# TritonDataCenter/dragnet

Hardware: AMD Instinct MI355X
Metric: NDJSON records/sec (whole node), krill filter + 2-field breakdown (req.method,res.statusCode) (higher is better)
Workload: dtype uint8; 1 GPU; model=dn scan: filter eq(req.method,GET) + breakdown req.method,res.statusCode, global_batch=4743501, seq_len=226, parallelism=dp1

## Files before the change

### dragnet_amd/ops/hip/scan_record.h

```cpp
#pragma once
#include "scan_text.h"

namespace dn {

constexpr int BLOCK = 256;
constexpr int SIG_DEPTH = 6;


struct FV {
  uint8_t* type;
  uint32_t* soff;
  uint32_t* slen;
  int tid;
  DN_HD_INLINE void set(int f, uint8_t t, uint32_t off, uint32_t len,
                        double n) {
    type[f * BLOCK + tid] = t;
    if (t == T_NUM) {
      uint64_t b = (uint64_t)DN_DOUBLE_AS_LL(n);
      soff[f * BLOCK + tid] = (uint32_t)b;
      slen[f * BLOCK + tid] = (uint32_t)(b >> 32);
    } else {
      soff[f * BLOCK + tid] = off;
      slen[f * BLOCK + tid] = len;
    }
  }
  DN_HD_INLINE void set_len(int f, uint32_t len) {
    slen[f * BLOCK + tid] = len;
  }
  DN_HD_INLINE uint8_t get_type(int f) const { return type[f * BLOCK + tid]; }
  DN_HD_INLINE uint32_t get_soff(int f) const { return soff[f * BLOCK + tid]; }
  DN_HD_INLINE uint32_t get_slen(int f) const { return slen[f * BLOCK + tid]; }
  DN_HD_INLINE double get_num(int f) const {
    uint64_t b = (uint64_t)soff[f * BLOCK + tid]
               | ((uint64_t)slen[f * BLOCK + tid] << 32);
    return DN_LL_AS_DOUBLE((long long)b);
  }
};


template <class BS>
DN_HD_INLINE bool parse_record(BS BV, uint32_t start, uint32_t end,
                               const PlanView& P, FV& fv, uint8_t& top_type,
                               uint64_t* sig_lds, bool dot_splits) {
  CursorT<BS> c; c.init(BV, start, end);
  #define sig_stack_at(d) sig_lds[(d) * BLOCK + DN_TID()]

  uint64_t cont_slot = ~0ull;
  uint64_t is_arr_bits = 0;
  int depth = 0;
  int arr_depth = 0;
  uint64_t cur_sig = 0;
  bool cur_capture = false;
  int cur_slot = -1;

  c.skip_ws();
  if (c.eof()) return false;

  auto match_slot = [&](uint64_t sig) -> int {
    if (!((P.sig_bloom >> ((uint32_t)sig & 63u)) & 1ull)) return -1;
    for (int f = 0; f < P.nf; f++)
      if (P.field_sigs[f] == sig) return f;
    return -1;
  };

  auto parse_key = [&](uint64_t parent, bool root, uint64_t& sig_out) -> bool {
    if (c.eof() || c.next() != '"') return false;
    int r = scan_key_sig(c, root ? FNV_OFFSET : parent, sig_out,
                         dot_splits);
    if (r == 0) return false;
    if (r == 2 && !root && parent == P.fields_parent_sig)
      sig_out = sig_mix(sig_out ^ SIG_LIT_MARK);
    return true;
  };

  bool expect_value = true;
  top_type = T_MISSING;

  while (true) {
    if (expect_value) {
      c.skip_ws();
      if (c.eof()) return false;
      uint8_t b = c.peek();
      uint8_t vtype = T_MISSING;
      uint32_t voff = 0, vlen = 0;
      double vnum = 0.0;

      if (b == '{') {
        uint32_t vstart = c.pos;
        c.pos++;
        if (cur_capture && arr_depth == 0)
          fv.set(cur_slot, T_OBJ, vstart, 0, 0.0);
        if (depth == 0) top_type = T_OBJ;
        if (depth >= MAX_DEPTH) return false;
        c.skip_ws();
        if (!c.eof() && c.peek() == '}') {
          c.pos++;
          vtype = T_OBJ;
          voff = vstart; vlen = c.pos - vstart;
        } else {
          if (depth < SLOT_DEPTH) {
            uint64_t cs = (cur_capture && arr_depth == 0)
                              ? (uint64_t)cur_slot : 31ull;
            cont_slot = (cont_slot & ~(31ull << (5 * depth)))
                        | (cs << (5 * depth));
          }
          if (depth < SIG_DEPTH) sig_stack_at(depth) = cur_sig;
          is_arr_bits &= ~(1ull << depth);
          depth++;
          uint64_t ksig;
          if (!parse_key(cur_sig, depth == 1, ksig)) return false;
          c.skip_ws();
          if (c.eof() || c.next() != ':') return false;
          cur_sig = ksig;
          cur_slot = (arr_depth == 0) ? match_slot(ksig) : -1;
          cur_capture = cur_slot >= 0;
          continue;
        }
      } else if (b == '[') {
        uint32_t vstart = c.pos;
        c.pos++;
        if (cur_capture && arr_depth == 0)
          fv.set(cur_slot, T_ARR, vstart, 0, 0.0);
        if (depth == 0) top_type = T_ARR;
        if (depth >= MAX_DEPTH) return false;
        c.skip_ws();
        if (!c.eof() && c.peek() == ']') {
          c.pos++;
          vtype = T_ARR;
          voff = vstart; vlen = c.pos - vstart;
        } else {
          if (depth < SLOT_DEPTH) {
            uint64_t cs = (cur_capture && arr_depth == 0)
                              ? (uint64_t)cur_slot : 31ull;
            cont_slot = (cont_slot & ~(31ull << (5 * depth)))
                        | (cs << (5 * depth));
          }
          if (depth < SIG_DEPTH) sig_stack_at(depth) = cur_sig;
          is_arr_bits |= (1ull << depth);
          depth++;
          arr_depth++;
          cur_capture = false; cur_slot = -1;
          continue;
        }
      } else if (b == '"') {
        c.pos++;
        if (!scan_string_fast(c, voff, vlen)) return false;
        vtype = T_STR;
      } else if (b == 't') {
        if (c.end - c.pos < 4) return false;
        if (c.byte_at(c.pos+1)!='r'||c.byte_at(c.pos+2)!='u'||c.byte_at(c.pos+3)!='e') return false;
        c.pos += 4; vtype = T_TRUE;
      } else if (b == 'f') {
        if (c.end - c.pos < 5) return false;
        if (c.byte_at(c.pos+1)!='a'||c.byte_at(c.pos+2)!='l'||c.byte_at(c.pos+3)!='s'||c.byte_at(c.pos+4)!='e') return false;
        c.pos += 5; vtype = T_FALSE;
      } else if (b == 'n') {
        if (c.end - c.pos < 4) return false;
        if (c.byte_at(c.pos+1)!='u'||c.byte_at(c.pos+2)!='l'||c.byte_at(c.pos+3)!='l') return false;
        c.pos += 4; vtype = T_NULL;
      } else if (b == '-' || (b >= '0' && b <= '9')) {
        NumOut n = parse_json_number(c);
        if (!n.ok) return false;
        vtype = T_NUM; vnum = n.v;
      } else {
        return false;
      }

      if (vtype != T_MISSING) {
        if (cur_capture && arr_depth == 0)
          fv.set(cur_slot, vtype, voff, vlen, vnum);
        if (depth == 0) { top_type = (top_type == T_MISSING) ? vtype : top_type; }
      }
      expect_value = false;
      continue;
    }

    if (depth == 0) {
      c.skip_ws();
      return c.eof();
    }
    c.skip_ws();
    if (c.eof()) return false;
    uint8_t b = c.next();
    bool in_arr = (is_arr_bits >> (depth - 1)) & 1u;
    if (in_arr) {
      if (b == ',') { expect_value = true; cur_capture = false; cur_slot = -1; continue; }
      if (b == ']') {
        depth--; arr_depth--;
        {
          int cs = (depth < SLOT_DEPTH)
                       ? (int)((cont_slot >> (5 * depth)) & 31ull) : 31;
          if (cs != 31) fv.set_len(cs, c.pos - fv.get_soff(cs));
        }
        cur_sig = (depth < SIG_DEPTH) ? sig_stack_at(depth) : 0;
        continue;
      }
      return false;
    } else {
      if (b == ',') {
        c.skip_ws();
        uint64_t parent = (depth - 1 < SIG_DEPTH) ? sig_stack_at(depth - 1) : 0;
        uint64_t ksig;
        if (!parse_key(parent, depth == 1, ksig)) return false;
        c.skip_ws();
        if (c.eof() || c.next() != ':') return false;
        cur_sig = ksig;
        cur_slot = (arr_depth == 0) ? match_slot(ksig) : -1;
        cur_capture = cur_slot >= 0;
        expect_value = true;
        continue;
      }
      if (b == '}') {
        depth--;
        {
          int cs = (depth < SLOT_DEPTH)
                       ? (int)((cont_slot >> (5 * depth)) & 31ull) : 31;
          if (cs != 31) fv.set_len(cs, c.pos - fv.get_soff(cs));
        }
        cur_sig = (depth < SIG_DEPTH) ? sig_stack_at(depth) : 0;
        continue;
      }
      return false;
    }
  }
}


template <class BS>
DN_HD_INLINE int eval_leaf(const PlanView& P, BS BV, const FV& fv,
                           int op, int slot, int cidx) {
  uint8_t ft = fv.get_type(slot);
  if (ft == T_MISSING) return -1;

  int ckind = P.const_meta[cidx * 6 + 0];
  uint32_t coff = (uint32_t)P.const_meta[cidx * 6 + 1];
  uint32_t clen = (uint32_t)P.const_meta[cidx * 6 + 2];
  int cdvalid = P.const_meta[cidx * 6 + 3];
  double cdval = P.const_dvals[cidx];

  if (op == OP_EQ || op == OP_NE) {
    bool eq = false;
    if (ft == T_NULL) {
      eq = (ckind == CONST_NULL);
    } else if (ckind == CONST_NULL) {
      eq = false;
    } else if (ft == T_TRUE || ft == T_FALSE || ft == T_NUM) {
      double fnum = (ft == T_NUM) ? fv.get_num(slot) : (ft == T_TRUE ? 1.0 : 0.0);
      if (ckind == CONST_NUM) eq = (fnum == cdval);
      else eq = cdvalid && (fnum == cdval);
    } else if (ft == T_STR) {
      if (ckind == CONST_STR) {
        uint32_t fo = fv.get_soff(slot), fl = fv.get_slen(slot);
        if (fl == clen) {
          eq = true;
          for (uint32_t k = 0; k < fl; k++)
            if (BV.at(fo + k) != P.const_bytes[coff + k]) { eq = false; break; }
        }
        if (!eq) {
          uint32_t co2 = (uint32_t)P.const_meta[cidx * 6 + 4];
          uint32_t cl2 = (uint32_t)P.const_meta[cidx * 6 + 5];
          if (cl2 != 0 && fl == cl2) {
            eq = true;
            for (uint32_t k = 0; k < fl; k++)
              if (BV.at(fo + k) != P.const_bytes[co2 + k]) { eq = false; break; }
          }
        }
        if (!eq && span_has_backslash(BV, fo, fl))
          eq = unesc_cmp(BV, fo, fl, P.const_bytes + coff, clen) == 0;
      } else {
        double fn = js_to_number(BV, fv.get_soff(slot), fv.get_slen(slot));
        eq = (fn == fn) && (fn == cdval);
      }
    } else {
      eq = false;
    }
    return (op == OP_EQ) ? (eq ? 1 : 0) : (eq ? 0 : 1);
  }

  if (ft == T_STR && ckind == CONST_STR) {
    uint32_t fo = fv.get_soff(slot), fl = fv.get_slen(slot);
    int cmp = 0;
    if (span_has_backslash(BV, fo, fl)) {
      cmp = unesc_cmp(BV, fo, fl, P.const_bytes + coff, clen);
      if (cmp == -2) cmp = 0;
    } else {
      uint32_t n = fl < clen ? fl : clen;
      for (uint32_t k = 0; k < n; k++) {
        uint8_t a = BV.at(fo + k), b = P.const_bytes[coff + k];
        if (a != b) { cmp = a < b ? -1 : 1; break; }
      }
      if (cmp == 0) cmp = (fl < clen) ? -1 : (fl > clen ? 1 : 0);
    }
    switch (op) {
      case OP_LT: return cmp < 0;
      case OP_LE: return cmp <= 0;
      case OP_GT: return cmp > 0;
      default:    return cmp >= 0;
    }
  }
  double x, y;
  if (ft == T_NUM) x = fv.get_num(slot);
  else if (ft == T_NULL) x = 0.0;
  else if (ft == T_TRUE) x = 1.0;
  else if (ft == T_FALSE) x = 0.0;
  else if (ft == T_STR) x = js_to_number(BV, fv.get_soff(slot), fv.get_slen(slot));
  else x = __builtin_nan("");
  if (ckind == CONST_NUM) y = cdval;
  else if (ckind == CONST_NULL) y = 0.0;
  else y = cdvalid ? cdval : __builtin_nan("");
  if (x != x || y != y) return 0;
  switch (op) {
    case OP_LT: return x < y;
    case OP_LE: return x <= y;
    case OP_GT: return x > y;
    default:    return x >= y;
  }
}

template <class BS>
DN_HD_INLINE int eval_predicate(const PlanView& P, BS BV,
                                const FV& fv, int prog_id) {
  int idx = P.prog_bounds[prog_id * 2 + 0];
  uint64_t stk[PRED_STACK];
  int sp = 0;
  int result;
  while (true) {
    int op = P.prog_nodes[idx * 4 + 0];
    if (op == OP_AND || op == OP_OR) {
      if (sp >= PRED_STACK) return -1;
      stk[sp] = ((uint64_t)(op == OP_OR)
                  | ((uint64_t)P.prog_nodes[idx * 4 + 1] << 1)
                  | ((uint64_t)P.prog_nodes[idx * 4 + 3] << 32));
      sp++;
      idx++;
      continue;
    }
    if (op == OP_TRUE) {
      result = 1;
      idx = P.prog_nodes[idx * 4 + 3];
    } else {
      result = eval_leaf(P, BV, fv, op,
                         P.prog_nodes[idx * 4 + 1],
                         P.prog_nodes[idx * 4 + 2]);
      idx = P.prog_nodes[idx * 4 + 3];
    }
    while (sp > 0) {
      if (result == -1) return -1;
      uint64_t f = stk[sp - 1];
      bool is_or = f & 1;
      uint32_t remaining = (uint32_t)(f >> 1) & 0x7FFFFF;
      bool sc = (!is_or && result == 0) || (is_or && result == 1);
      remaining--;
      if (sc || remaining == 0) {
        idx = (int)(f >> 32);
        sp--;
      } else {
        stk[sp - 1] = (f & 0xFFFFFFFF00000001ull)
                      | ((uint64_t)remaining << 1);
        break;
      }
    }
    if (sp == 0) return result;
  }
}

}
```

### dragnet_amd/ops/hip/scan_text.h

```cpp
#pragma once
#include "common.h"
#include "dec2dbl.h"

namespace dn {


DN_HD_INLINE uint64_t fnv1a_byte(uint64_t h, uint8_t b) {
  return (h ^ (uint64_t)b) * 0x100000001B3ull;
}
constexpr uint64_t FNV_OFFSET = 0xCBF29CE484222325ull;

DN_CONST_TABLE double P10_TBL[23] = {
  1e0,1e1,1e2,1e3,1e4,1e5,1e6,1e7,1e8,1e9,1e10,1e11,1e12,1e13,1e14,
  1e15,1e16,1e17,1e18,1e19,1e20,1e21,1e22};
DN_CONST_TABLE int DIM_TBL[12] = {
  31,28,31,30,31,30,31,31,30,31,30,31};

DN_HD_INLINE uint64_t mix64(uint64_t x) {
  x ^= x >> 33; x *= 0xFF51AFD7ED558CCDull;
  x ^= x >> 33; x *= 0xC4CEB9FE1A85EC53ull;
  x ^= x >> 33; return x;
}


struct Bytes {
  const uint8_t* mem;
  uint32_t bias;
  DN_HD_INLINE uint8_t at(uint32_t abs) const { return mem[abs - bias]; }
  DN_HD_INLINE uint64_t load8(uint32_t abs) const {
    uint64_t w;
    __builtin_memcpy(&w, mem + (abs - bias), 8);
    return w;
  }
};

template <int LG>
struct XBytesT {
  static constexpr uint32_t GRAN = 1u << LG;
  static constexpr uint32_t STRIDE = 64u << LG;
  const uint8_t* base;
  DN_HD_INLINE uint8_t at(uint32_t p) const {
    return base[(size_t)(p >> LG) * STRIDE + (p & (GRAN - 1u))];
  }
  DN_HD_INLINE uint64_t load8(uint32_t p) const {
    uint32_t o = p & (GRAN - 1u);
    const uint8_t* gp = base + (size_t)(p >> LG) * STRIDE;
    uint64_t w;
    if (o <= GRAN - 8) {
      __builtin_memcpy(&w, gp + o, 8);
      return w;
    }
    uint64_t lo, hi;
    __builtin_memcpy(&lo, gp + GRAN - 8, 8);
    __builtin_memcpy(&hi, gp + STRIDE, 8);
    uint32_t sh = (o - (GRAN - 8)) * 8;
    return (lo >> sh) | (hi << (64 - sh));
  }
};

template <class BS>
struct CursorT {
  BS B;
  uint32_t pos, end;
  uint64_t win, win2;
  uint32_t wbase;

  DN_HD_INLINE void init(BS b, uint32_t p, uint32_t e) {
    B = b; pos = p; end = e;
    wbase = p;
    win = B.load8(p);
    win2 = B.load8(p + 8);
  }
  DN_HD_INLINE uint8_t byte_at(uint32_t p) {
    uint32_t d = p - wbase;
    if (d >= 16u) {
      wbase = p;
      win = B.load8(p);
      win2 = B.load8(p + 8);
      d = 0;
    }
    uint64_t w = d < 8u ? win : win2;
    return (uint8_t)(w >> (8u * (d & 7u)));
  }
  DN_HD_INLINE bool eof() const { return pos >= end; }
  DN_HD_INLINE uint8_t peek() { return byte_at(pos); }
  DN_HD_INLINE uint8_t next() { return byte_at(pos++); }
  DN_HD_INLINE uint64_t word_at(uint32_t p) {
    uint32_t d = p - wbase;
    if (d > 8u) {
      wbase = p;
      win = B.load8(p);
      win2 = B.load8(p + 8);
      d = 0;
    }
    if (d == 0) return win;
    if (d == 8u) return win2;
    return (win >> (8u * d)) | (win2 << (64u - 8u * d));
  }
  DN_HD_INLINE void skip_ws() {
    while (pos < end) {
      uint8_t b = byte_at(pos);
      if (b == ' ' || b == '\t' || b == '\r' || b == '\n') pos++;
      else break;
    }
  }
};

DN_HD_INLINE uint64_t hz8(uint64_t v) {
  return (v - 0x0101010101010101ull) & ~v & 0x8080808080808080ull;
}

DN_HD_INLINE uint64_t str_special_mask(uint64_t w) {
  uint64_t q = hz8(w ^ 0x2222222222222222ull);
  uint64_t b = hz8(w ^ 0x5C5C5C5C5C5C5C5Cull);
  uint64_t c = hz8(w & 0xE0E0E0E0E0E0E0E0ull);
  return q | b | c;
}

template <class BS>
DN_HD_INLINE bool scan_string_fast(CursorT<BS>& c, uint32_t& off_out,
                                   uint32_t& len_out) {
  uint32_t off = c.pos, p = c.pos, end = c.end;
  while (true) {
    while (p + 8 <= end) {
      uint64_t w = c.B.load8(p);
      uint64_t m = str_special_mask(w);
      if (m == 0) { p += 8; continue; }
      p += ((uint32_t)DN_FFSLL((unsigned long long)m) - 1) >> 3;
      break;
    }
    if (p >= end) return false;
    uint8_t b = c.B.at(p);
    if (b == '"') {
      off_out = off; len_out = p - off; c.pos = p + 1;
      return true;
    }
    if (b == '\\') {
      p++;
      if (p >= end) return false;
      uint8_t e = c.B.at(p); p++;
      if (e == 'u') {
        if (p + 4 > end) return false;
        for (int k = 0; k < 4; k++) {
          uint8_t x = c.B.at(p + k);
          bool hex = (x >= '0' && x <= '9') || (x >= 'a' && x <= 'f') ||
                     (x >= 'A' && x <= 'F');
          if (!hex) return false;
        }
        p += 4;
      } else if (!(e == '"' || e == '\\' || e == '/' || e == 'b' ||
                   e == 'f' || e == 'n' || e == 'r' || e == 't')) {
        return false;
      }
      continue;
    }
    if (b < 0x20) return false;
    p++;
  }
}

constexpr uint64_t SIG_LENK = 0xFF51AFD7ED558CCDull;

DN_HD_INLINE uint64_t sig_mix(uint64_t x) {
  x ^= x >> 32;
  x *= 0xD6E8FEB86659FD93ull;
  return x ^ (x >> 32);
}
constexpr uint64_t SIG_LIT_MARK = 0xC2B2AE3D27D4EB4Full;

DN_HD_INLINE uint64_t sig_word(uint64_t sig, uint64_t w) {
  return sig_mix(sig ^ w);
}
DN_HD_INLINE uint64_t sig_fin(uint64_t sig, uint32_t len) {
  return sig_mix(sig ^ ((uint64_t)len * SIG_LENK));
}

template <class BS>
DN_HD_INLINE uint64_t sig_comp_finish(BS B, uint64_t sig, uint32_t hashed,
                                      uint32_t comp_s, uint32_t term) {
  uint32_t k = hashed;
  while (k < term) {
    uint64_t w = B.load8(k);
    uint32_t rem = term - k;
    if (rem < 8) w &= (~0ull) >> (8 * (8 - rem));
    sig = sig_mix(sig ^ w);
    k += 8;
  }
  return sig_fin(sig, term - comp_s);
}

template <class BS>
DN_HD_INLINE int scan_key_sig(CursorT<BS>& c, uint64_t parent,
                              uint64_t& sig_out, bool dot_splits) {
  uint32_t p = c.pos, end = c.end;
  uint32_t comp_s = p;
  uint32_t hashed = p;
  uint64_t sig = parent;
  bool saw_dot = false;
  while (true) {
    while (p + 8 <= end) {
      uint64_t w = c.B.load8(p);
      uint64_t m = str_special_mask(w);
      if (dot_splits) m |= hz8(w ^ 0x2E2E2E2E2E2E2E2Eull);
      if (m == 0) {
        if (p == hashed) {
          sig = sig_word(sig, w);
          hashed = p + 8;
        }
        p += 8;
        continue;
      }
      p += ((uint32_t)DN_FFSLL((unsigned long long)m) - 1) >> 3;
      break;
    }
    if (p >= end) return 0;
    uint8_t b = c.B.at(p);
    if (b == '"') {
      sig_out = sig_comp_finish(c.B, sig, hashed, comp_s, p);
      c.pos = p + 1;
      return saw_dot ? 2 : 1;
    }
    if (b == '.') {
      if (dot_splits) {
        sig = sig_comp_finish(c.B, sig, hashed, comp_s, p);
        comp_s = p + 1;
        hashed = p + 1;
        saw_dot = true;
      }
      p++;
      continue;
    }
    if (b == '\\') {
      c.pos = p;
      uint32_t o, l;
      if (!scan_string_fast(c, o, l)) return 0;
      sig_out = 0x1ull;
      return 1;
    }
    if (b < 0x20) return 0;
    p++;
  }
}


DN_HD_INLINE double scale10(uint64_t mant, long ex) {
  return dn_dec2dbl(mant, ex, P10_TBL);
}

struct NumOut { double v; bool ok; };

template <class BS>
DN_HD_INLINE int scan_digit_run(CursorT<BS>& c, uint64_t& mant, int& ndig,
                                int& extra) {
  int total = 0;
  while (!c.eof()) {
    uint64_t w = c.word_at(c.pos);
    uint64_t t = w ^ 0x3030303030303030ull;
    uint64_t nd = ((t + 0x7676767676767676ull) | t)
                  & 0x8080808080808080ull;
    uint32_t n = nd ? (((uint32_t)DN_FFSLL((long long)nd) - 1) >> 3)
                    : 8u;
    uint32_t avail = c.end - c.pos;
    if (n > avail) n = avail;
    if (n == 0) break;
    if (n == 8 && mant != 0 && ndig + 8 <= 19) {
      uint64_t pairs = (t * ((10ull << 8) + 1)) >> 8;
      uint64_t quads = ((pairs & 0x00FF00FF00FF00FFull)
                        * ((100ull << 16) + 1)) >> 16;
      uint64_t v8 = ((quads & 0x0000FFFF0000FFFFull)
                     * ((10000ull << 32) + 1)) >> 32;
      mant = mant * 100000000ull + (uint32_t)v8;
      ndig += 8;
    } else {
      for (uint32_t k = 0; k < n; k++) {
        uint32_t d = (uint32_t)(w >> (8 * k)) & 0xFF;
        if (ndig < 19) {
          mant = mant * 10u + (d - '0');
          ndig += (mant != 0);
        } else extra++;
      }
    }
    c.pos += n;
    total += (int)n;
    if (n < 8) break;
  }
  return total;
}

template <class BS>
DN_HD_INLINE NumOut parse_json_number(CursorT<BS>& c) {
  NumOut out; out.ok = false; out.v = 0.0;
  bool neg = false;
  if (!c.eof() && c.peek() == '-') { neg = true; c.pos++; }
  if (c.eof()) return out;
  uint64_t mant = 0;
  int ndig = 0, extra_exp = 0;
  uint8_t b = c.peek();
  if (b == '0') {
    c.pos++;
    if (!c.eof()) { uint8_t nb = c.peek(); if (nb >= '0' && nb <= '9') return out; }
  } else if (b >= '1' && b <= '9') {
    scan_digit_run(c, mant, ndig, extra_exp);
  } else {
    return out;
  }
  if (!c.eof() && c.peek() == '.') {
    c.pos++;
    int fdig = 0, fex = 0;
    fdig = scan_digit_run(c, mant, ndig, fex);
    extra_exp -= (fdig - fex);
    if (fdig == 0) return out;
  }
  int esign = 1; long e10 = 0;
  if (!c.eof() && (c.peek() == 'e' || c.peek() == 'E')) {
    c.pos++;
    if (!c.eof() && (c.peek() == '+' || c.peek() == '-')) {
      if (c.peek() == '-') esign = -1;
      c.pos++;
    }
    int edig = 0;
    while (!c.eof()) {
      uint8_t d = c.peek();
      if (d < '0' || d > '9') break;
      c.pos++;
      if (e10 < 100000) e10 = e10 * 10 + (d - '0');
      edig++;
    }
    if (edig == 0) return out;
  }
  long exp10 = esign * e10 + extra_exp;
  double v = scale10(mant, exp10);
  out.v = neg ? -v : v;
  out.ok = true;
  return out;
}

DN_HD_INLINE bool raw_ws(uint8_t b) {
  return b == ' ' || b == '\t' || b == '\r' || b == '\n' || b == '\f' ||
         b == '\v';
}

template <class BS>
DN_HD_INLINE uint32_t ws_escape_at(BS BV, uint32_t off, uint32_t p, uint32_t j,
                                   bool py_ws) {
  if (p + 2 > j || BV.at(off + p) != '\\') return 0;
  uint8_t e = BV.at(off + p + 1);
  if (e == 't' || e == 'n' || e == 'r' || e == 'f') return 2;
  if (e != 'u' || p + 6 > j) return 0;
  uint32_t cp = 0;
  for (int k = 2; k < 6; k++) {
    uint8_t x = BV.at(off + p + k);
    uint32_t d;
    if (x >= '0' && x <= '9') d = x - '0';
    else if (x >= 'a' && x <= 'f') d = x - 'a' + 10;
    else if (x >= 'A' && x <= 'F') d = x - 'A' + 10;
    else return 0;
    cp = cp * 16 + d;
  }
  bool ws = (cp >= 0x09 && cp <= 0x0D) || cp == 0x20 || cp == 0xA0 ||
            cp == 0x1680 || (cp >= 0x2000 && cp <= 0x200A) ||
            cp == 0x2028 || cp == 0x2029 || cp == 0x202F ||
            cp == 0x205F || cp == 0x3000 ||
            (py_ws ? ((cp >= 0x1C && cp <= 0x1F) || cp == 0x85)
                   : cp == 0xFEFF);
  return ws ? 6u : 0u;
}

template <class BS>
DN_HD_INLINE uint64_t trim_escaped_ws(BS BV, uint32_t off, uint32_t i,
                                      uint32_t j, bool py_ws) {
  while (i < j) {
    if (raw_ws(BV.at(off + i))) { i++; continue; }
    uint32_t n = ws_escape_at(BV, off, i, j, py_ws);
    if (n == 0) break;
    i += n;
  }
  while (j > i) {
    if (raw_ws(BV.at(off + j - 1))) { j--; continue; }
    uint32_t n = 0;
    if (j - i >= 2 && ws_escape_at(BV, off, j - 2, j, py_ws) == 2) n = 2;
    else if (j - i >= 6 && ws_escape_at(BV, off, j - 6, j, py_ws) == 6) n = 6;
    if (n == 0) break;
    uint32_t run = 0;
    for (uint32_t k = j - n; k > i && BV.at(off + k - 1) == '\\'; k--) run++;
    if (run & 1) break;
    j -= n;
  }
  return (uint64_t)i | ((uint64_t)j << 32);
}

template <class BS>
DN_HD_INLINE void trim_ws(BS BV, uint32_t off, uint32_t& i, uint32_t& j,
                          bool py_ws) {
  while (i < j && raw_ws(BV.at(off + i))) i++;
  while (j > i && raw_ws(BV.at(off + j - 1))) j--;
  if (j - i >= 2 &&
      (BV.at(off + i) == '\\' || BV.at(off + j - 2) == '\\' ||
       (j - i >= 6 && BV.at(off + j - 6) == '\\')))
  {
    uint64_t ij = trim_escaped_ws(BV, off, i, j, py_ws);
    i = (uint32_t)ij;
    j = (uint32_t)(ij >> 32);
  }
}

template <class BS>
DN_HD_INLINE double js_to_number(BS BV, uint32_t off, uint32_t len) {
  uint32_t i = 0, j = len;
  trim_ws(BV, off, i, j, false);
  if (i == j) return 0.0;
  const double NAN_ = __builtin_nan("");
  uint32_t p = i;
  bool neg = false;
  if (BV.at(off+p) == '+' || BV.at(off+p) == '-') { neg = BV.at(off+p) == '-'; p++; }
  if (p == j) return NAN_;
  if (BV.at(off+p) == 'I') {
    const char* inf = "Infinity";
    if (j - p == 8) {
      for (int k = 0; k < 8; k++) if (BV.at(off+p+k) != (uint8_t)inf[k]) return NAN_;
      return neg ? -__builtin_inf() : __builtin_inf();
    }
    return NAN_;
  }
  if (j - p > 2 && BV.at(off+p) == '0' &&
      (BV.at(off+p+1) == 'x' || BV.at(off+p+1) == 'X')) {
    if (p != i) return NAN_;
    uint64_t v = 0; int shift4 = 0; bool sticky = false;
    for (uint32_t k = p + 2; k < j; k++) {
      uint8_t b = BV.at(off+k);
      uint32_t d;
      if (b >= '0' && b <= '9') d = b - '0';
      else if (b >= 'a' && b <= 'f') d = b - 'a' + 10;
      else if (b >= 'A' && b <= 'F') d = b - 'A' + 10;
      else return NAN_;
      if (v >> 60) { shift4++; sticky |= (d != 0); }
      else v = v * 16u + d;
    }
    if (sticky) v |= 1;
    double r = (double)v;
    for (; shift4 > 0 && r < __builtin_inf(); shift4--) r *= 16.0;
    return r;
  }
  uint64_t mant = 0; int ndig = 0, extra = 0; bool any = false;
  while (p < j && BV.at(off+p) >= '0' && BV.at(off+p) <= '9') {
    if (ndig < 19) { mant = mant * 10 + (BV.at(off+p)-'0'); ndig += (mant != 0); }
    else extra++;
    p++; any = true;
  }
  if (p < j && BV.at(off+p) == '.') {
    p++;
    while (p < j && BV.at(off+p) >= '0' && BV.at(off+p) <= '9') {
      if (ndig < 19) { mant = mant * 10 + (BV.at(off+p)-'0'); ndig += (mant != 0); extra--; }
      p++; any = true;
    }
  }
  if (!any) return NAN_;
  long e10 = 0; int es = 1;
  if (p < j && (BV.at(off+p) == 'e' || BV.at(off+p) == 'E')) {
    p++;
    if (p < j && (BV.at(off+p) == '+' || BV.at(off+p) == '-')) {
      if (BV.at(off+p) == '-') es = -1;
      p++;
    }
    if (p >= j) return NAN_;
    while (p < j && BV.at(off+p) >= '0' && BV.at(off+p) <= '9') {
      if (e10 < 100000) e10 = e10 * 10 + (BV.at(off+p)-'0');
      p++;
    }
  }
  if (p != j) return NAN_;
  long ex = es * e10 + extra;
  double v = scale10(mant, ex);
  return neg ? -v : v;
}


DN_HD_INLINE bool finite_num(double v) {
  return __builtin_fabs(v) < __builtin_inf();
}

DN_HD_INLINE double bucket_ordinal(int kind, double num, double step) {
  if (kind == BUCKET_P2) {
    if (!(num >= 1.0)) return 0.0;
    uint64_t bits = DN_DOUBLE_AS_LL(num);
    return (double)((int)((bits >> 52) & 0x7FF) - 1023 + 1);
  }
  return __builtin_floor(num / step);
}

DN_HD_INLINE bool ord_is_small(double ordf) {
  return ordf >= -(double)ORD_BIAS && ordf < (double)ORD_BIAS;
}


DN_HD_INLINE long days_from_civil(long y, long m, long d) {
  y -= m <= 2;
  long era = (y >= 0 ? y : y - 399) / 400;
  long yoe = y - era * 400;
  long doy = (153 * (m + (m > 2 ? -3 : 9)) + 2) / 5 + d - 1;
  long doe = yoe * 365 + yoe / 4 - yoe / 100 + doy;
  return era * 146097 + doe - 719468;
}

struct DateOut { long long ms; bool ok; };

DN_HD_INLINE bool is_leap(long y) {
  return (y % 4 == 0) && ((y % 100 != 0) || (y % 400 == 0));
}

template <class BS>
DN_HD_INLINE DateOut parse_iso_ms(BS BV, uint32_t off, uint32_t len) {
  DateOut out; out.ok = false; out.ms = 0;
  uint32_t i = 0, j = len;
  trim_ws(BV, off, i, j, true);
  uint32_t p = i;
  auto digits = [&](int n, long& v) -> bool {
    v = 0;
    for (int k = 0; k < n; k++) {
      if (p >= j) return false;
      uint8_t b = BV.at(off+p);
      if (b < '0' || b > '9') return false;
      v = v * 10 + (b - '0');
      p++;
    }
    return true;
  };
  long year, month = 1, day = 1, hh = 0, mm = 0, ss = 0, ms = 0;
  if (!digits(4, year)) return out;
  bool have_time = false;
  if (p < j && BV.at(off+p) == '-') {
    p++;
    if (!digits(2, month)) return out;
    if (p < j && BV.at(off+p) == '-') {
      p++;
      if (!digits(2, day)) return out;
      if (p < j && (BV.at(off+p) == 'T' || BV.at(off+p) == ' ')) {
        p++;
        if (!digits(2, hh)) return out;
        if (p >= j || BV.at(off+p) != ':') return out;
        p++;
        if (!digits(2, mm)) return out;
        have_time = true;
        if (p < j && BV.at(off+p) == ':') {
          p++;
          if (!digits(2, ss)) return out;
          if (p < j && BV.at(off+p) == '.') {
            p++;
            int nd = 0; long frac = 0;
            while (p < j && BV.at(off+p) >= '0' && BV.at(off+p) <= '9' && nd < 9) {
              if (nd < 3) frac = frac * 10 + (BV.at(off+p) - '0');
              nd++; p++;
            }
            if (nd == 0) return out;
            while (nd < 3) { frac *= 10; nd++; }
            ms = frac;
          }
        }
      }
    }
  }
  long tz_off_min = 0;
  if (have_time && p < j) {
    uint8_t b = BV.at(off+p);
    if (b == 'Z') { p++; }
    else if (b == '+' || b == '-') {
      int sign = (b == '+') ? 1 : -1;
      p++;
      long th, tm;
      if (!digits(2, th)) return out;
      if (p < j && BV.at(off+p) == ':') p++;
      if (!digits(2, tm)) return out;
      tz_off_min = sign * (th * 60 + tm);
    }
  }
  if (p != j) return out;
  if (month < 1 || month > 12) return out;
  long dim = DIM_TBL[month-1] + ((month == 2 && is_leap(year)) ? 1 : 0);
  if (day < 1 || day > dim) return out;
  if (hh > 24 || mm > 59 || ss > 59) return out;
  if (hh == 24 && (mm || ss || ms)) return out;
  long days = days_from_civil(year, month, day);
  long long total = ((days * 24 + hh) * 60 + mm) * 60 + ss;
  out.ms = total * 1000 + ms - (long long)tz_off_min * 60000;
  out.ok = true;
  return out;
}


DN_HD_INLINE int hexval4(uint8_t x) {
  if (x >= '0' && x <= '9') return x - '0';
  if (x >= 'a' && x <= 'f') return x - 'a' + 10;
  if (x >= 'A' && x <= 'F') return x - 'A' + 10;
  return -1;
}

template <class BS>
DN_HD_INLINE int unesc_next(BS d, uint32_t fo, uint32_t fl,
                            uint32_t& i, uint32_t& out) {
  uint8_t b = d.at(fo + i);
  if (b != '\\') { i++; out = b; return 1; }
  if (i + 2 > fl) return 0;
  uint8_t e = d.at(fo + i + 1);
  i += 2;
  switch (e) {
    case '"':  out = '"';  return 1;
    case '\\': out = '\\'; return 1;
    case '/':  out = '/';  return 1;
    case 'b':  out = 8;    return 1;
    case 'f':  out = 12;   return 1;
    case 'n':  out = 10;   return 1;
    case 'r':  out = 13;   return 1;
    case 't':  out = 9;    return 1;
    case 'u':  break;
    default:   return 0;
  }
  if (i + 4 > fl) return 0;
  uint32_t cp = 0;
  for (int k = 0; k < 4; k++) {
    int h = hexval4(d.at(fo + i + k));
    if (h < 0) return 0;
    cp = cp * 16 + (uint32_t)h;
  }
  i += 4;
  if (cp >= 0xD800 && cp < 0xDC00 && i + 6 <= fl &&
      d.at(fo + i) == '\\' && d.at(fo + i + 1) == 'u') {
    uint32_t lo = 0;
    bool ok = true;
    for (int k = 0; k < 4; k++) {
      int h = hexval4(d.at(fo + i + 2 + k));
      if (h < 0) { ok = false; break; }
      lo = lo * 16 + (uint32_t)h;
    }
    if (ok && lo >= 0xDC00 && lo < 0xE000) {
      cp = 0x10000 + ((cp - 0xD800) << 10) + (lo - 0xDC00);
      i += 6;
    }
  }
  if (cp < 0x80) { out = cp; return 1; }
  if (cp < 0x800) {
    out = (0xC0 | (cp >> 6)) | ((0x80u | (cp & 63)) << 8);
    return 2;
  }
  if (cp < 0x10000) {
    out = (0xE0 | (cp >> 12)) | ((0x80u | ((cp >> 6) & 63)) << 8)
          | ((0x80u | (cp & 63)) << 16);
    return 3;
  }
  out = (0xF0 | (cp >> 18)) | ((0x80u | ((cp >> 12) & 63)) << 8)
        | ((0x80u | ((cp >> 6) & 63)) << 16)
        | ((0x80u | (cp & 63)) << 24);
  return 4;
}

template <class BS>
DN_HD_INLINE int unesc_cmp(BS d, uint32_t fo, uint32_t fl,
                           const uint8_t* cb, uint32_t cl) {
  uint32_t i = 0, j = 0;
  while (i < fl) {
    uint32_t pack;
    int n = unesc_next(d, fo, fl, i, pack);
    if (n == 0) return -2;
    for (int k = 0; k < n; k++) {
      uint8_t a = (uint8_t)(pack >> (8 * k));
      if (j >= cl) return 1;
      uint8_t b = cb[j++];
      if (a != b) return a < b ? -1 : 1;
    }
  }
  return (j == cl) ? 0 : -1;
}

template <class BS>
DN_HD_INLINE bool span_has_backslash(BS d, uint32_t fo, uint32_t fl) {
  for (uint32_t k = 0; k < fl; k++)
    if (d.at(fo + k) == '\\') return true;
  return false;
}

}
```

### tools_dev/kernel_host_check.cpp

```cpp
#include <cinttypes>
#include <cstdio>
#include <cstdlib>
#include <cstring>
#include <iostream>
#include <sstream>
#include <string>
#include <vector>

#include "scan_record.h"

using namespace dn;

static uint64_t bits_of(double v) {
  uint64_t b;
  std::memcpy(&b, &v, 8);
  return b;
}

static std::string unhex(const std::string& h) {
  std::string out;
  if (h == "-") return out;
  for (size_t i = 0; i + 1 < h.size(); i += 2)
    out.push_back((char)std::stoi(h.substr(i, 2), nullptr, 16));
  return out;
}

template <class BS> struct Staged;

template <> struct Staged<Bytes> {
  uint8_t* buf;
  Bytes src;
  explicit Staged(const std::string& rec) {
    size_t n = rec.size() + 1;
    size_t padded = (n + 16 + 15) & ~(size_t)15;
    buf = (uint8_t*)std::malloc(padded);
    std::memset(buf, '\n', padded);
    std::memcpy(buf, rec.data(), rec.size());
    src.mem = buf;
    src.bias = 0;
  }
  ~Staged() { std::free(buf); }
};

template <int LG> struct Staged<XBytesT<LG>> {
  uint8_t* buf;
  XBytesT<LG> src;
  explicit Staged(const std::string& rec) {
    const size_t GRAN = XBytesT<LG>::GRAN, STRIDE = XBytesT<LG>::STRIDE;
    size_t rows = (rec.size() + GRAN - 1) / GRAN;
    if (rows == 0) rows = 1;
    size_t total = rows * STRIDE + STRIDE;
    buf = (uint8_t*)std::malloc(total);
    std::memset(buf, '\n', total);
    for (size_t p = 0; p < rec.size(); p++)
      buf[(p >> LG) * STRIDE + (p & (GRAN - 1))] = (uint8_t)rec[p];
    src.base = buf;
  }
  ~Staged() { std::free(buf); }
};

struct Plan {
  std::vector<uint64_t> field_sigs;
  std::vector<int32_t> prog_nodes, prog_bounds, const_meta;
  std::vector<double> const_dvals;
  std::vector<uint8_t> const_bytes;
  bool dot_splits = false;
  PlanView P;
  std::vector<uint8_t> fv_type;
  std::vector<uint32_t> fv_soff, fv_slen;
  std::vector<uint64_t> sig_stack;

  void bind() {
    P.field_sigs = field_sigs.data();
    P.prog_nodes = prog_nodes.data();
    P.prog_bounds = prog_bounds.data();
    P.const_meta = const_meta.data();
    P.const_dvals = const_dvals.data();
    P.const_bytes = const_bytes.data();
    fv_type.assign((size_t)P.nf * BLOCK, T_MISSING);
    fv_soff.assign((size_t)P.nf * BLOCK, 0);
    fv_slen.assign((size_t)P.nf * BLOCK, 0);
    sig_stack.assign((size_t)SIG_DEPTH * BLOCK, 0);
  }
};

template <class BS>
static void do_record(Plan& pl, const std::string& rec) {
  Staged<BS> st(rec);
  pl.bind();
  FV fv;
  fv.type = pl.fv_type.data();
  fv.soff = pl.fv_soff.data();
  fv.slen = pl.fv_slen.data();
  fv.tid = 0;
  uint8_t top = T_MISSING;
  bool ok = parse_record(st.src, 0u, (uint32_t)rec.size(), pl.P, fv, top,
                         pl.sig_stack.data(), pl.dot_splits);
  if (!ok) { std::printf("0\n"); return; }
  std::printf("1 %d", (int)top);
  for (int f = 0; f < pl.P.nf; f++) {
    int t = fv.get_type(f);
    if (t == T_NUM)
      std::printf(" 4:%016" PRIx64, bits_of(fv.get_num(f)));
    else if (t == T_STR || t == T_OBJ || t == T_ARR)
      std::printf(" %d:%u:%u", t, fv.get_soff(f), fv.get_slen(f));
    else
      std::printf(" %d", t);
  }
  std::printf(" ;");
  int nprogs = (int)pl.prog_bounds.size() / 2;
  for (int p = 0; p < nprogs; p++)
    std::printf(" %d", eval_predicate(pl.P, st.src, fv, p));
  std::printf("\n");
}

template <class BS>
static int serve() {
  Plan pl;
  std::memset(&pl.P, 0, sizeof(pl.P));
  std::string line, mode, tok;
  while (std::getline(std::cin, line)) {
    std::istringstream in(line);
    if (!(in >> mode)) continue;
    if (mode == "dec2dbl") {
      unsigned long long mant; long ex;
      in >> mant >> ex;
      std::printf("%016" PRIx64 "\n",
                  bits_of(dn_dec2dbl((uint64_t)mant, ex, P10_TBL)));
    } else if (mode == "number") {
      in >> tok;
      std::string lit = unhex(tok);
      Staged<BS> st(lit);
      CursorT<BS> c;
      c.init(st.src, 0u, (uint32_t)lit.size());
      NumOut n = parse_json_number(c);
      std::printf("%s %016" PRIx64 " %u\n",
                  n.ok && c.pos == c.end ? "ok" : "invalid", bits_of(n.v),
                  c.pos);
    } else if (mode == "tonumber") {
      in >> tok;
      std::string s = unhex(tok);
      Staged<BS> st(s);
      std::printf("%016" PRIx64 "\n",
                  bits_of(js_to_number(st.src, 0u, (uint32_t)s.size())));
    } else if (mode == "date") {
      in >> tok;
      std::string s = unhex(tok);
      Staged<BS> st(s);
      DateOut d = parse_iso_ms(st.src, 0u, (uint32_t)s.size());
      if (d.ok) std::printf("ok %lld\n", d.ms);
      else std::printf("invalid\n");
    } else if (mode == "keysig") {
      int dot_splits;
      in >> dot_splits;
      uint64_t sig = FNV_OFFSET;
      bool ok = true;
      while (ok && (in >> tok)) {
        std::string key = unhex(tok) + "\"";
        Staged<BS> st(key);
        CursorT<BS> c;
        c.init(st.src, 0u, (uint32_t)key.size());
        uint64_t out = 0;
        ok = scan_key_sig(c, sig, out, dot_splits != 0) != 0;
        sig = out;
      }
      if (ok) std::printf("%016" PRIx64 "\n", sig);
      else std::printf("invalid\n");
    } else if (mode == "plan") {
      int ds;
      std::string bloom, fps;
      in >> ds >> pl.P.nf >> bloom >> fps;
      pl.dot_splits = ds != 0;
      pl.P.sig_bloom = std::stoull(bloom, nullptr, 16);
      pl.P.fields_parent_sig = std::stoull(fps, nullptr, 16);
    } else if (mode == "field_sigs") {
      pl.field_sigs.clear();
      while (in >> tok) pl.field_sigs.push_back(std::stoull(tok, nullptr, 16));
    } else if (mode == "const_dvals") {
      pl.const_dvals.clear();
      while (in >> tok) {
        uint64_t b = std::stoull(tok, nullptr, 16);
        double v;
        std::memcpy(&v, &b, 8);
        pl.const_dvals.push_back(v);
      }
    } else if (mode == "const_bytes") {
      in >> tok;
      std::string b = unhex(tok);
      pl.const_bytes.assign(b.begin(), b.end());
    } else if (mode == "prog_nodes" || mode == "prog_bounds" ||
               mode == "const_meta") {
      std::vector<int32_t>& v = mode == "prog_nodes" ? pl.prog_nodes
                              : mode == "prog_bounds" ? pl.prog_bounds
                                                      : pl.const_meta;
      v.clear();
      long x;
      while (in >> x) v.push_back((int32_t)x);
    } else if (mode == "record") {
      tok = "-";
      in >> tok;
      do_record<BS>(pl, unhex(tok));
    } else {
      std::fprintf(stderr, "unknown request: %s\n", mode.c_str());
      return 2;
    }
  }
  return 0;
}

int main(int argc, char** argv) {
  std::string src = argc > 1 ? argv[1] : "bytes";
  if (src == "bytes") return serve<Bytes>();
  if (src == "x5") return serve<XBytesT<5>>();
  if (src == "x6") return serve<XBytesT<6>>();
  if (src == "x7") return serve<XBytesT<7>>();
  std::fprintf(stderr, "usage: kernel_host_check <bytes|x5|x6|x7>\n");
  return 2;
}
```

Measured before the change: 248.4 million records/s.

## Rewrite JSON record parser as word-at-a-time SWAR state machine

```diff
diff --git a/dragnet_amd/ops/hip/scan_record.h b/dragnet_amd/ops/hip/scan_record.h
--- a/dragnet_amd/ops/hip/scan_record.h
+++ b/dragnet_amd/ops/hip/scan_record.h
@@ -38,11 +38,25 @@
 };
 
 
+enum ParseState : uint32_t {
+  PS_VALUE = 0,
+  PS_ELEM1,
+  PS_KEYC,
+  PS_KEY,
+  PS_COLON,
+  PS_AFTER,
+  PS_STR,
+  PS_KEYB,
+  PS_NUMS,
+  PS_NUM0,
+  PS_NUM,
+};
+
 template <class BS>
 DN_HD_INLINE bool parse_record(BS BV, uint32_t start, uint32_t end,
                                const PlanView& P, FV& fv, uint8_t& top_type,
-                               uint64_t* sig_lds, bool dot_splits) {
-  CursorT<BS> c; c.init(BV, start, end);
+                               uint64_t* sig_lds, bool dot_splits,
+                               uint32_t* trips = nullptr) {
   #define sig_stack_at(d) sig_lds[(d) * BLOCK + DN_TID()]
 
   uint64_t cont_slot = ~0ull;
@@ -50,179 +64,305 @@
   int depth = 0;
   int arr_depth = 0;
   uint64_t cur_sig = 0;
-  bool cur_capture = false;
   int cur_slot = -1;
-
-  c.skip_ws();
-  if (c.eof()) return false;
+  uint32_t st = PS_VALUE;
+  uint32_t pos = start;
+  uint32_t tok_off = start;
+  uint64_t kacc = 0;
+  uint32_t kn = 0;
+  bool saw_dot = false;
+  top_type = T_MISSING;
 
   auto match_slot = [&](uint64_t sig) -> int {
     if (!((P.sig_bloom >> ((uint32_t)sig & 63u)) & 1ull)) return -1;
-    for (int f = 0; f < P.nf; f++)
-      if (P.field_sigs[f] == sig) return f;
-    return -1;
+    int slot = -1;
+    for (int f = P.nf - 1; f >= 0; f--)
+      if (P.field_sigs[f] == sig) slot = f;
+    return slot;
   };
 
-  auto parse_key = [&](uint64_t parent, bool root, uint64_t& sig_out) -> bool {
-    if (c.eof() || c.next() != '"') return false;
-    int r = scan_key_sig(c, root ? FNV_OFFSET : parent, sig_out,
-                         dot_splits);
-    if (r == 0) return false;
-    if (r == 2 && !root && parent == P.fields_parent_sig)
-      sig_out = sig_mix(sig_out ^ SIG_LIT_MARK);
-    return true;
+  auto close_container = [&](bool in_arr, uint32_t end_pos) {
+    depth--;
+    if (in_arr) arr_depth--;
+    int cs = (depth < SLOT_DEPTH)
+                 ? (int)((cont_slot >> (5 * depth)) & 31ull) : 31;
+    if (cs != 31) fv.set_len(cs, end_pos - fv.get_soff(cs));
+    cur_sig = (depth < SIG_DEPTH) ? sig_stack_at(depth) : 0;
   };
 
-  bool expect_value = true;
-  top_type = T_MISSING;
-
-  while (true) {
-    if (expect_value) {
-      c.skip_ws();
-      if (c.eof()) return false;
-      uint8_t b = c.peek();
-      uint8_t vtype = T_MISSING;
-      uint32_t voff = 0, vlen = 0;
-      double vnum = 0.0;
-
-      if (b == '{') {
-        uint32_t vstart = c.pos;
-        c.pos++;
-        if (cur_capture && arr_depth == 0)
-          fv.set(cur_slot, T_OBJ, vstart, 0, 0.0);
-        if (depth == 0) top_type = T_OBJ;
+  for (;;) {
+    if (trips) ++*trips;
+    uint32_t avail = end - pos;
+    uint64_t w = BV.load8(pos);
+    if (avail < 8u) {
+      uint64_t keep = sw_low(avail);
+      w = (w & keep) | (0x0A0A0A0A0A0A0A0Aull & ~keep);
+    }
+    uint32_t o = 0;
+    bool fresh = false;
+    bool neg = false;
+    bool key_done = false, colon_done = false;
+    uint32_t nx = 8;
+    uint8_t vtype = T_MISSING;
+    uint32_t voff = 0, vlen = 0;
+    double vnum = 0.0;
+
+    if (st < PS_STR) {
+      uint64_t nonws = sw_stops(w, SW_WS);
+      uint32_t k = sw_first(nonws, 0);
+      if (sw_bad_ws(w, k < avail ? k : avail)) return false;
+      if (k >= avail) return st == PS_AFTER && depth == 0;
+      if (k == 8u) { pos += 8u; continue; }
+      uint8_t b = (uint8_t)(w >> (8u * k));
+
+      bool sep = false;
+      if (st == PS_AFTER) {
+        if (depth == 0) return false;
+        bool in_arr = (is_arr_bits >> (depth - 1)) & 1u;
+        if (b == ',') {
+          if (in_arr) { st = PS_VALUE; cur_slot = -1; }
+          else st = PS_KEY;
+          sep = true;
+        } else if (b == (in_arr ? ']' : '}')) {
+          close_container(in_arr, pos + k + 1);
+          pos += k + 1;
+          continue;
+        } else {
+          return false;
+        }
+      } else if (st == PS_COLON) {
+        if (b != ':') return false;
+        st = PS_VALUE;
+        sep = true;
+      } else if (st == PS_VALUE && (b == '{' || b == '[')) {
+        uint8_t t = (b == '{') ? T_OBJ : T_ARR;
+        if (cur_slot >= 0 && arr_depth == 0)
+          fv.set(cur_slot, t, pos + k, 0, 0.0);
+        if (depth == 0) top_type = t;
         if (depth >= MAX_DEPTH) return false;
-        c.skip_ws();
-        if (!c.eof() && c.peek() == '}') {
-          c.pos++;
+        st = (b == '{') ? PS_KEYC : PS_ELEM1;
+        tok_off = pos + k;
+        sep = true;
+      }
+      if (sep) {
+        uint32_t k2 = sw_first(nonws, k + 1u);
+        uint64_t w2 = (w & ~(0xFFull << (8u * k))) | (0x20ull << (8u * k));
+        if (sw_bad_ws(w2, k2 < avail ? k2 : avail)) return false;
+        if (k2 >= avail) return false;
+        if (k2 == 8u) { pos += 8u; continue; }
+        k = k2;
+        b = (uint8_t)(w >> (8u * k));
+      }
+      uint32_t at = pos + k;
+
+      if (st == PS_KEYC || st == PS_KEY) {
+        if (st == PS_KEYC && b == '}') {
           vtype = T_OBJ;
-          voff = vstart; vlen = c.pos - vstart;
+          voff = tok_off; vlen = at + 1 - tok_off;
+          pos = at + 1;
         } else {
-          if (depth < SLOT_DEPTH) {
-            uint64_t cs = (cur_capture && arr_depth == 0)
-                              ? (uint64_t)cur_slot : 31ull;
-            cont_slot = (cont_slot & ~(31ull << (5 * depth)))
-                        | (cs << (5 * depth));
-          }
-          if (depth < SIG_DEPTH) sig_stack_at(depth) = cur_sig;
-          is_arr_bits &= ~(1ull << depth);
-          depth++;
-          uint64_t ksig;
-          if (!parse_key(cur_sig, depth == 1, ksig)) return false;
-          c.skip_ws();
-          if (c.eof() || c.next() != ':') return false;
-          cur_sig = ksig;
-          cur_slot = (arr_depth == 0) ? match_slot(ksig) : -1;
-          cur_capture = cur_slot >= 0;
+          if (b != '"') return false;
+          uint64_t parent;
+          if (st == PS_KEYC) {
+            if (depth < SLOT_DEPTH) {
+              uint64_t cs = (cur_slot >= 0 && arr_depth == 0)
+                                ? (uint64_t)cur_slot : 31ull;
+              cont_slot = (cont_slot & ~(31ull << (5 * depth)))
+                          | (cs << (5 * depth));
+            }
+            if (depth < SIG_DEPTH) sig_stack_at(depth) = cur_sig;
+            is_arr_bits &= ~(1ull << depth);
+            depth++;
+            parent = cur_sig;
+          } else {
+            parent = (depth - 1 < SIG_DEPTH) ? sig_stack_at(depth - 1) : 0;
+          }
+          cur_sig = (depth == 1) ? FNV_OFFSET : parent;
+          kacc = 0; kn = 0; saw_dot = false;
+          st = PS_KEYB;
+          tok_off = at + 1;
+          o = k + 1;
+        }
+      } else {
+        if (st == PS_ELEM1) {
+          if (b == ']') {
+            vtype = T_ARR;
+            voff = tok_off; vlen = at + 1 - tok_off;
+            pos = at + 1;
+          } else {
+            if (depth < SLOT_DEPTH) {
+              uint64_t cs = (cur_slot >= 0 && arr_depth == 0)
+                                ? (uint64_t)cur_slot : 31ull;
+              cont_slot = (cont_slot & ~(31ull << (5 * depth)))
+                          | (cs << (5 * depth));
+            }
+            if (depth < SIG_DEPTH) sig_stack_at(depth) = cur_sig;
+            is_arr_bits |= (1ull << depth);
+            depth++;
+            arr_depth++;
+            cur_slot = -1;
+            st = PS_VALUE;
+          }
+        }
+        if (st == PS_VALUE) {
+          if (b == '{' || b == '[') {
+            pos = at;
+            continue;
+          } else if (b == '"') {
+            st = PS_STR;
+            tok_off = at + 1;
+            o = k + 1;
+          } else if (b == '-' || (b >= '0' && b <= '9')) {
+            st = PS_NUMS;
+            fresh = true;
+            neg = (b == '-');
+            tok_off = at;
+            o = k + (neg ? 1u : 0u);
+          } else if (b == 't' || b == 'f' || b == 'n') {
+            uint32_t len = (b == 'f') ? 5u : 4u;
+            if (avail - k < len) return false;
+            uint64_t lw = k ? BV.load8(at) : w;
+            uint64_t want = (b == 't') ? 0x65757274ull
+                          : (b == 'f') ? 0x65736C6166ull : 0x6C6C756Eull;
+            if ((lw & sw_low(len)) != want) return false;
+            vtype = (b == 't') ? T_TRUE : (b == 'f') ? T_FALSE : T_NULL;
+            pos = at + len;
+          } else {
+            return false;
+          }
+        }
+      }
+    }
+
+    if (st >= PS_STR) {
+      bool isnum = st >= PS_NUMS;
+      uint64_t stops = sw_stops(w, SW_STR);
+      if (dot_splits && st == PS_KEYB)
+        stops |= ~sw_nz(w ^ 0x2E2E2E2E2E2E2E2Eull) & SW_H8;
+      if (isnum) stops = sw_stops(w, SW_DIGIT);
+      uint32_t e = sw_first(stops, o);
+      uint32_t n = e - o;
+      uint8_t sb = (e < 8u) ? (uint8_t)(w >> (8u * e)) : 0;
+
+      if (!isnum) {
+        if (st == PS_KEYB) {
+          uint64_t nb = n ? ((w >> (8u * o)) & sw_low(n)) : 0;
+          uint64_t comb = kacc | (nb << (8u * kn));
+          if (kn + n >= 8u) {
+            cur_sig = sig_word(cur_sig, comb);
+            kacc = kn ? (nb >> (8u * (8u - kn))) : 0;
+            kn = kn + n - 8u;
+          } else {
+            kacc = comb;
+            kn += n;
+          }
+        }
+        if (e == 8u) { pos += 8u; continue; }
+        if (sb == '"') {
+          if (st == PS_KEYB) {
+            if (kn) cur_sig = sig_word(cur_sig, kacc);
+            cur_sig = sig_fin(cur_sig, pos + e - tok_off);
+            if (saw_dot && depth != 1) {
+              uint64_t parent =
+                  (depth - 1 < SIG_DEPTH) ? sig_stack_at(depth - 1) : 0;
+              if (parent == P.fields_parent_sig)
+                cur_sig = sig_mix(cur_sig ^ SIG_LIT_MARK);
+            }
+            key_done = true;
+            if (e < 7u && (uint8_t)(w >> (8u * (e + 1u))) == ':') {
+              colon_done = true;
+              pos++;
+            }
+          } else {
+            vtype = T_STR;
+            voff = tok_off; vlen = pos + e - tok_off;
+            nx = e + 1u;
+          }
+          pos += e + 1u;
+        } else if (sb == '.') {
+          if (kn) cur_sig = sig_word(cur_sig, kacc);
+          cur_sig = sig_fin(cur_sig, pos + e - tok_off);
+          kacc = 0; kn = 0; saw_dot = true;
+          pos += e + 1u;
+          tok_off = pos;
           continue;
-        }
-      } else if (b == '[') {
-        uint32_t vstart = c.pos;
-        c.pos++;
-        if (cur_capture && arr_depth == 0)
-          fv.set(cur_slot, T_ARR, vstart, 0, 0.0);
-        if (depth == 0) top_type = T_ARR;
-        if (depth >= MAX_DEPTH) return false;
-        c.skip_ws();
-        if (!c.eof() && c.peek() == ']') {
-          c.pos++;
-          vtype = T_ARR;
-          voff = vstart; vlen = c.pos - vstart;
+        } else if (sb == '\\') {
+          CursorT<BS> c; c.init(BV, pos + e, end);
+          uint32_t so, sl;
+          if (!scan_string_fast(c, so, sl)) return false;
+          pos = c.pos;
+          if (st == PS_KEYB) {
+            cur_sig = 0x1ull;
+            key_done = true;
+          } else {
+            vtype = T_STR;
+            voff = tok_off; vlen = pos - 1u - tok_off;
+          }
         } else {
-          if (depth < SLOT_DEPTH) {
-            uint64_t cs = (cur_capture && arr_depth == 0)
-                              ? (uint64_t)cur_slot : 31ull;
-            cont_slot = (cont_slot & ~(31ull << (5 * depth)))
-                        | (cs << (5 * depth));
-          }
-          if (depth < SIG_DEPTH) sig_stack_at(depth) = cur_sig;
-          is_arr_bits |= (1ull << depth);
-          depth++;
-          arr_depth++;
-          cur_capture = false; cur_slot = -1;
+          return false;
+        }
+        if (key_done) {
+          cur_slot = (arr_depth == 0) ? match_slot(cur_sig) : -1;
+          st = colon_done ? PS_VALUE : PS_COLON;
           continue;
         }
-      } else if (b == '"') {
-        c.pos++;
-        if (!scan_string_fast(c, voff, vlen)) return false;
-        vtype = T_STR;
-      } else if (b == 't') {
-        if (c.end - c.pos < 4) return false;
-        if (c.byte_at(c.pos+1)!='r'||c.byte_at(c.pos+2)!='u'||c.byte_at(c.pos+3)!='e') return false;
-        c.pos += 4; vtype = T_TRUE;
-      } else if (b == 'f') {
-        if (c.end - c.pos < 5) return false;
-        if (c.byte_at(c.pos+1)!='a'||c.byte_at(c.pos+2)!='l'||c.byte_at(c.pos+3)!='s'||c.byte_at(c.pos+4)!='e') return false;
-        c.pos += 5; vtype = T_FALSE;
-      } else if (b == 'n') {
-        if (c.end - c.pos < 4) return false;
-        if (c.byte_at(c.pos+1)!='u'||c.byte_at(c.pos+2)!='l'||c.byte_at(c.pos+3)!='l') return false;
-        c.pos += 4; vtype = T_NULL;
-      } else if (b == '-' || (b >= '0' && b <= '9')) {
-        NumOut n = parse_json_number(c);
-        if (!n.ok) return false;
-        vtype = T_NUM; vnum = n.v;
       } else {
-        return false;
-      }
-
-      if (vtype != T_MISSING) {
-        if (cur_capture && arr_depth == 0)
-          fv.set(cur_slot, vtype, voff, vlen, vnum);
-        if (depth == 0) { top_type = (top_type == T_MISSING) ? vtype : top_type; }
-      }
-      expect_value = false;
-      continue;
-    }
-
-    if (depth == 0) {
-      c.skip_ws();
-      return c.eof();
-    }
-    c.skip_ws();
-    if (c.eof()) return false;
-    uint8_t b = c.next();
-    bool in_arr = (is_arr_bits >> (depth - 1)) & 1u;
-    if (in_arr) {
-      if (b == ',') { expect_value = true; cur_capture = false; cur_slot = -1; continue; }
-      if (b == ']') {
-        depth--; arr_depth--;
-        {
-          int cs = (depth < SLOT_DEPTH)
-                       ? (int)((cont_slot >> (5 * depth)) & 31ull) : 31;
-          if (cs != 31) fv.set_len(cs, c.pos - fv.get_soff(cs));
-        }
-        cur_sig = (depth < SIG_DEPTH) ? sig_stack_at(depth) : 0;
-        continue;
-      }
-      return false;
-    } else {
-      if (b == ',') {
-        c.skip_ws();
-        uint64_t parent = (depth - 1 < SIG_DEPTH) ? sig_stack_at(depth - 1) : 0;
-        uint64_t ksig;
-        if (!parse_key(parent, depth == 1, ksig)) return false;
-        c.skip_ws();
-        if (c.eof() || c.next() != ':') return false;
-        cur_sig = ksig;
-        cur_slot = (arr_depth == 0) ? match_slot(ksig) : -1;
-        cur_capture = cur_slot >= 0;
-        expect_value = true;
-        continue;
-      }
-      if (b == '}') {
-        depth--;
-        {
-          int cs = (depth < SLOT_DEPTH)
-                       ? (int)((cont_slot >> (5 * depth)) & 31ull) : 31;
-          if (cs != 31) fv.set_len(cs, c.pos - fv.get_soff(cs));
-        }
-        cur_sig = (depth < SIG_DEPTH) ? sig_stack_at(depth) : 0;
-        continue;
-      }
-      return false;
-    }
-  }
+        if (st == PS_NUMS) {
+          if (n == 0) {
+            if (e < 8u) return false;
+          } else if ((uint8_t)(w >> (8u * o)) == '0') {
+            if (n > 1u) return false;
+            st = PS_NUM0;
+          } else {
+            st = PS_NUM;
+          }
+        } else if (st == PS_NUM0) {
+          if (n) return false;
+        }
+        if (e == 8u) { pos += 8u; continue; }
+        bool need = (cur_slot >= 0 && arr_depth == 0) || depth == 0;
+        if (sb == '.' || sb == 'e' || sb == 'E' || (need && !fresh)) {
+          CursorT<BS> c; c.init(BV, tok_off, end);
+          NumOut r = parse_json_number(c, need);
+          if (!r.ok) return false;
+          vnum = r.v;
+          pos = c.pos;
+        } else {
+          if (need) {
+            uint64_t t = w ^ 0x3030303030303030ull;
+            double v = (double)fold8_digits((t >> (8u * o))
+                                            << (8u * (8u - n)));
+            vnum = neg ? -v : v;
+          }
+          pos += e;
+          nx = e;
+        }
+        vtype = T_NUM;
+      }
+    }
+
+    if (cur_slot >= 0 && arr_depth == 0)
+      fv.set(cur_slot, vtype, voff, vlen, vnum);
+    if (depth == 0 && top_type == T_MISSING) top_type = vtype;
+    st = PS_AFTER;
+    if (nx < 8u && depth > 0) {
+      uint8_t nb = (uint8_t)(w >> (8u * nx));
+      bool in_arr = (is_arr_bits >> (depth - 1)) & 1u;
+      if (nb == (in_arr ? ']' : '}')) {
+        pos++;
+        close_container(in_arr, pos);
+        nx++;
+        nb = (nx < 8u) ? (uint8_t)(w >> (8u * nx)) : 0;
+        in_arr = depth > 0 && ((is_arr_bits >> (depth - 1)) & 1u);
+      }
+      if (nb == ',' && depth > 0) {
+        if (in_arr) { st = PS_VALUE; cur_slot = -1; }
+        else st = PS_KEY;
+        pos++;
+      }
+    }
+  }
+  #undef sig_stack_at
 }
 
 
diff --git a/dragnet_amd/ops/hip/scan_text.h b/dragnet_amd/ops/hip/scan_text.h
--- a/dragnet_amd/ops/hip/scan_text.h
+++ b/dragnet_amd/ops/hip/scan_text.h
@@ -84,7 +84,6 @@
   }
   DN_HD_INLINE bool eof() const { return pos >= end; }
   DN_HD_INLINE uint8_t peek() { return byte_at(pos); }
-  DN_HD_INLINE uint8_t next() { return byte_at(pos++); }
   DN_HD_INLINE uint64_t word_at(uint32_t p) {
     uint32_t d = p - wbase;
     if (d > 8u) {
@@ -97,13 +96,6 @@
     if (d == 8u) return win2;
     return (win >> (8u * d)) | (win2 << (64u - 8u * d));
   }
-  DN_HD_INLINE void skip_ws() {
-    while (pos < end) {
-      uint8_t b = byte_at(pos);
-      if (b == ' ' || b == '\t' || b == '\r' || b == '\n') pos++;
-      else break;
-    }
-  }
 };
 
 DN_HD_INLINE uint64_t hz8(uint64_t v) {
@@ -115,6 +107,56 @@
   uint64_t b = hz8(w ^ 0x5C5C5C5C5C5C5C5Cull);
   uint64_t c = hz8(w & 0xE0E0E0E0E0E0E0E0ull);
   return q | b | c;
+}
+
+constexpr uint64_t SW_L7 = 0x7F7F7F7F7F7F7F7Full;
+constexpr uint64_t SW_H8 = 0x8080808080808080ull;
+
+DN_HD_INLINE uint64_t sw_nz(uint64_t v) { return ((v & SW_L7) + SW_L7) | v; }
+
+enum SwClass : uint32_t { SW_WS = 0, SW_STR = 1, SW_DIGIT = 2 };
+
+DN_HD_INLINE uint64_t sw_stops(uint64_t w, uint32_t cls) {
+  if (cls == SW_WS)
+    return (((w & SW_L7) + 0x5F5F5F5F5F5F5F5Full) | w) & SW_H8;
+  if (cls == SW_DIGIT) {
+    uint64_t t = w ^ 0x3030303030303030ull;
+    return (((t & SW_L7) + 0x7676767676767676ull) | t) & SW_H8;
+  }
+  uint64_t run = sw_nz(w ^ 0x2222222222222222ull)
+               & sw_nz(w ^ 0x5C5C5C5C5C5C5C5Cull)
+               & sw_nz(w & 0xE0E0E0E0E0E0E0E0ull);
+  return ~run & SW_H8;
+}
+
+DN_HD_INLINE uint32_t sw_first(uint64_t stops, uint32_t from) {
+  if (from >= 8u) return 8u;
+  stops &= ~0ull << (8u * from);
+  return stops ? (((uint32_t)DN_FFSLL((unsigned long long)stops) - 1) >> 3)
+               : 8u;
+}
+
+DN_HD_INLINE uint64_t sw_low(uint32_t n) {
+  return n >= 8u ? ~0ull : ((1ull << (8u * n)) - 1);
+}
+
+DN_HD_INLINE bool sw_bad_ws(uint64_t w, uint32_t n) {
+  uint64_t m = sw_low(n);
+  if (((w ^ 0x2020202020202020ull) & m) == 0) return false;
+  uint64_t nonws = sw_nz(w ^ 0x2020202020202020ull)
+                 & sw_nz(w ^ 0x0909090909090909ull)
+                 & sw_nz(w ^ 0x0A0A0A0A0A0A0A0Aull)
+                 & sw_nz(w ^ 0x0D0D0D0D0D0D0D0Dull) & SW_H8;
+  return (nonws & m) != 0;
+}
+
+DN_HD_INLINE uint32_t fold8_digits(uint64_t t) {
+  uint64_t pairs = (t * ((10ull << 8) + 1)) >> 8;
+  uint64_t quads = ((pairs & 0x00FF00FF00FF00FFull)
+                    * ((100ull << 16) + 1)) >> 16;
+  uint64_t v8 = ((quads & 0x0000FFFF0000FFFFull)
+                 * ((10000ull << 32) + 1)) >> 32;
+  return (uint32_t)v8;
 }
 
 template <class BS>
@@ -264,12 +306,7 @@
     if (n > avail) n = avail;
     if (n == 0) break;
     if (n == 8 && mant != 0 && ndig + 8 <= 19) {
-      uint64_t pairs = (t * ((10ull << 8) + 1)) >> 8;
-      uint64_t quads = ((pairs & 0x00FF00FF00FF00FFull)
-                        * ((100ull << 16) + 1)) >> 16;
-      uint64_t v8 = ((quads & 0x0000FFFF0000FFFFull)
-                     * ((10000ull << 32) + 1)) >> 32;
-      mant = mant * 100000000ull + (uint32_t)v8;
+      mant = mant * 100000000ull + fold8_digits(t);
       ndig += 8;
     } else {
       for (uint32_t k = 0; k < n; k++) {
@@ -288,7 +325,8 @@
 }
 
 template <class BS>
-DN_HD_INLINE NumOut parse_json_number(CursorT<BS>& c) {
+DN_HD_INLINE NumOut parse_json_number(CursorT<BS>& c,
+                                      bool want_value = true) {
   NumOut out; out.ok = false; out.v = 0.0;
   bool neg = false;
   if (!c.eof() && c.peek() == '-') { neg = true; c.pos++; }
@@ -328,10 +366,11 @@
     }
     if (edig == 0) return out;
   }
+  out.ok = true;
+  if (!want_value) return out;
   long exp10 = esign * e10 + extra_exp;
   double v = scale10(mant, exp10);
   out.v = neg ? -v : v;
-  out.ok = true;
   return out;
 }
 
diff --git a/tools_dev/kernel_host_check.cpp b/tools_dev/kernel_host_check.cpp
--- a/tools_dev/kernel_host_check.cpp
+++ b/tools_dev/kernel_host_check.cpp
@@ -85,7 +85,8 @@
 };
 
 template <class BS>
-static void do_record(Plan& pl, const std::string& rec) {
+static void do_record(Plan& pl, const std::string& rec,
+                      bool count_trips = false) {
   Staged<BS> st(rec);
   pl.bind();
   FV fv;
@@ -94,8 +95,10 @@
   fv.slen = pl.fv_slen.data();
   fv.tid = 0;
   uint8_t top = T_MISSING;
+  uint32_t trips = 0;
   bool ok = parse_record(st.src, 0u, (uint32_t)rec.size(), pl.P, fv, top,
-                         pl.sig_stack.data(), pl.dot_splits);
+                         pl.sig_stack.data(), pl.dot_splits, &trips);
+  if (count_trips) { std::printf("%d %u\n", ok ? 1 : 0, trips); return; }
   if (!ok) { std::printf("0\n"); return; }
   std::printf("1 %d", (int)top);
   for (int f = 0; f < pl.P.nf; f++) {
@@ -196,10 +199,10 @@
       v.clear();
       long x;
       while (in >> x) v.push_back((int32_t)x);
-    } else if (mode == "record") {
+    } else if (mode == "record" || mode == "trips") {
       tok = "-";
       in >> tok;
-      do_record<BS>(pl, unhex(tok));
+      do_record<BS>(pl, unhex(tok), mode == "trips");
     } else {
       std::fprintf(stderr, "unknown request: %s\n", mode.c_str());
       return 2;
```

Measured after the change: 247.7 million records/s. Within noise of the previous version (-0.2%).
